# bcgsc/NanoSim

Measured on AMD Instinct MI355X. Metric: simulated reads/sec (genome mode, mean 8 kb), higher is better.
Workload: dtype u8

## Files before the change

nanosim_amd/csrc/nanosim_amd.hip:

```cpp
#include <hip/hip_runtime.h>
#include <hipcub/hipcub.hpp>
#include <stdio.h>
#include <stdlib.h>
#include <string.h>
#include <algorithm>
#include <chrono>
#include <atomic>
#include <condition_variable>
#include <functional>
#include <mutex>
#include <thread>
#include <string>
#include <vector>

#include "ns_device.h"
#include "ns_materialise.h"
#include "ns_chain.h"
#include "ns_hp.h"
#include "ns_ir.h"
#include "ns_io.h"
#include "ns_pack.h"
#include "ns_cs_hist.h"

#ifndef NS_WPB
// ... 3044 lines not shown
            continue;
        }
        pl.tot_cap = cap;
        break;
    }
    A.pieces = (ns_piece *)ctx->pieces.p;
    A.key_pos = (const uint32_t *)ctx->key_pos.p;
    pl.tot_pieces = n;
    info->ms_kernel[NS_K_EVENTS] = ms_chain;
    if (A.ir_need && (rc = ir_splice(ctx, A, n))) return rc;
    if (A.hp && (rc = hp_stage1(ctx, prm, A, n, pl.tot_pieces, stats, &pl.ms_hp))) return rc;
    return NS_OK;
}

static int genome_passes(ns_ctx *ctx, const ns_params *prm, ns_batch_info *info, GenArgs &A, Plan &pl) {
    const size_t n = (size_t)prm->n_reads;
    const Knobs &kn = ctx->knob;
    hipStream_t st = ctx->stream;
    unsigned long long *stats = pl.stats;
    uint32_t *list_a = (uint32_t *)ctx->order.p, *list_b = (uint32_t *)ctx->list_b.p, *list_c = (uint32_t *)ctx->list_c.p;
    const dim3 blk(256), grid_t((unsigned)((n + 1 + 255) / 256));
    const bool lds = ctx->lds_tables && prm->kind != NS_KIND_PERFECT;
    const bool chim_al = prm->kind == NS_KIND_ALIGNED && prm->chimeric;
    int rc;
    A.cap_rate = ctx->cap_rate;
    for (int hp_round = 0;; ++hp_round) {
        for (int retry = 0;; ++retry) {
            HIPCHK(hipMemsetAsync(ctx->stats.p, 0, NS_STATS_BYTES, st));
            HIPCHK(hipEventRecord(ctx->evt[1], st));
            k_nseg<<<grid_t, blk, 0, st>>>(A);
            HIPCHK(hipGetLastError());
            if ((rc = scan_u32(ctx, A.n_pieces, A.piece_off, n + 1))) return rc;
            if (chim_al) {
                uint32_t tp32 = 0;
                if ((rc = read_small(ctx, st, &tp32, A.piece_off + n, 4))) return rc;
                pl.tot_pieces = tp32;
            } else pl.tot_pieces = n;
            if ((rc = ensure(ctx, ctx->pieces, (size_t)pl.tot_pieces * sizeof(ns_piece) + 64))) return rc;
            A.pieces = (ns_piece *)ctx->pieces.p;
            A.list = nullptr; A.list_n = (uint32_t)n; A.attempt = 0;
            k_lengths<false><<<grid_t, blk, 0, st>>>(A);
            HIPCHK(hipGetLastError());
            if ((rc = scan_u64(ctx, A.ev_cap, A.ev_off, n + 1))) return rc;
            if ((rc = visiting_order(ctx, A.sort_key, A.sort_idx, n, list_a))) return rc;
            HIPCHK(hipEventRecord(ctx->evt[2], st));
            uint32_t n_multi = 0;
            if (prm->chimeric && prm->kind == NS_KIND_ALIGNED && ctx->ord_bins.p && !kn.exact_order) {
                if ((rc = read_small(ctx, st, &pl.tot_cap, A.ev_off + n, 8, &n_multi, (uint32_t *)ctx->ord_bins.p + 2 * NS_ORD_BINS, 4))) return rc;
            } else if ((rc = read_small(ctx, st, &pl.tot_cap, A.ev_off + n, 8))) return rc;
            if ((rc = ensure(ctx, ctx->events, (size_t)pl.tot_cap * sizeof(ns_event) + 64))) return rc;
            A.events = (ns_event *)ctx->events.p;
            uint32_t *cur = list_a, *nxt = list_b;
            uint32_t cur_n = (uint32_t)n;
            bool overflow = false;
            double ms_chain = 0;
            uint64_t used = pl.tot_cap;
            for (uint32_t a = 0;; ++a) {
                A.list = cur; A.list_n = cur_n; A.attempt = a; A.next_list = nxt; A.hole_at = 0; A.hole_len = 0; A.prio_thr = nullptr;
                A.l_off = nullptr; A.l_base = 0;
                if (a > 0) HIPCHK(hipMemsetAsync(A.next_n, 0, 4, st));
                const dim3 grid_p((cur_n + 255) / 256);
                A.p_need = nullptr; A.p_off = nullptr; A.p_base = 0;
                if (a > 0) {
                    if (chim_al) {
                        if ((rc = ensure_all(ctx, {{ctx->p_need, ((size_t)cur_n + 1) * 4}, {ctx->p_off, ((size_t)cur_n + 1) * 4}}))) return rc;
                        k_replan<<<dim3((cur_n + 1 + 255) / 256), blk, 0, st>>>(A, (uint32_t *)ctx->p_need.p);
                        HIPCHK(hipGetLastError());
                        if ((rc = scan_u32(ctx, (const uint32_t *)ctx->p_need.p, (uint32_t *)ctx->p_off.p, (size_t)cur_n + 1))) return rc;
                        uint32_t extra = 0;
                        if ((rc = read_small(ctx, st, &extra, (uint32_t *)ctx->p_off.p + cur_n, 4))) return rc;
                        if (extra) {
                            if ((rc = ensure_keep(ctx, ctx->pieces, (size_t)(pl.tot_pieces + extra) * sizeof(ns_piece) + 64,
                                                  (size_t)pl.tot_pieces * sizeof(ns_piece)))) return rc;
                            A.pieces = (ns_piece *)ctx->pieces.p;
                            A.p_need = (const uint32_t *)ctx->p_need.p; A.p_off = (const uint32_t *)ctx->p_off.p; A.p_base = (uint32_t)pl.tot_pieces;
                            pl.tot_pieces += extra;
                        }
                    }
                    if (cur_n <= 4096u) k_lengths<true><<<dim3((cur_n + 63) / 64), dim3(64), 0, st>>>(A);
                    else k_lengths<false><<<grid_p, blk, 0, st>>>(A);
                    HIPCHK(hipGetLastError());
                    HIPCHK(hipMemsetAsync(A.l_cap + cur_n, 0, 8, st));
                    if ((rc = scan_u64(ctx, A.l_cap, (uint64_t *)ctx->l_off.p, (size_t)cur_n + 1))) return rc;
                    uint64_t pass_cap = 0;
                    if ((rc = read_small(ctx, st, &pass_cap, (uint64_t *)ctx->l_off.p + cur_n, 8))) return rc;
                    if ((rc = ensure_keep(ctx, ctx->events, (size_t)(used + pass_cap) * sizeof(ns_event) + 64, (size_t)used * sizeof(ns_event)))) return rc;
                    A.events = (ns_event *)ctx->events.p;
                    A.l_off = (const uint64_t *)ctx->l_off.p; A.l_base = used;
                    used += pass_cap;
                }
                if (a == 0 && ctx->gate_wait) {
                    const auto t_end = std::chrono::steady_clock::now() + std::chrono::milliseconds(3);
                    while (!ctx->gate_wait->load(std::memory_order_acquire) && std::chrono::steady_clock::now() < t_end)
                        std::this_thread::yield();
                }
                HIPCHK(hipEventRecord(ctx->evt[3], st));
                uint32_t n_coop = 0;
                if (prm->kind == NS_KIND_UNALIGNED)
                    n_coop = (a == 0 && lds && cur_n >= kn.coop_min) ? std::max(cur_n >> kn.ucoop_shift, 1u) : cur_n;
                else if (a == 0 && ctx->coop_ok && prm->kind == NS_KIND_ALIGNED && cur_n >= kn.coop_min)
                    n_coop = (cur_n - std::min(cur_n, n_multi)) >> kn.coop_shift;
                const uint32_t coop_at = (a == 0 && prm->kind == NS_KIND_ALIGNED) ? std::min(cur_n, n_multi) : 0u;
                uint32_t m_coop = 0;
                if (coop_at && n_coop) {
                    const bool piece_threads = lds && !kn.no_piece_threads;
                    const uint32_t sh = piece_threads ? (kn.coop_shift > 1u ? kn.coop_shift - 1u : 0u) : (kn.coop_shift > 5u ? kn.coop_shift - 5u : 0u);
                    m_coop = std::min(coop_at, std::max(coop_at >> sh, 64u));
                }
                if (n_coop) {
                    GenArgs B = A; B.list_n = n_coop + m_coop; B.list = cur + (m_coop ? 0u : coop_at);
                    if (m_coop) { B.hole_at = m_coop; B.hole_len = coop_at - m_coop; }
                    B.coop_k1 = kn.ucoop_k1 ? 1u : 0u;
                    if ((rc = launch_chain_coop(ctx, B, st))) return rc;
                    if (coop_at) { A.list = cur + m_coop; A.hole_at = coop_at - m_coop; A.hole_len = n_coop; } else A.list = cur + n_coop;
                    A.list_n = cur_n - n_coop - m_coop;
                }
                uint32_t n_pt = 0;
                if (a == 0 && lds && n_coop && coop_at > m_coop && !kn.no_piece_threads) {
                    if (!ctx->stream3) {
                        HIPCHK(hipStreamCreateWithFlags(&ctx->stream3, hipStreamNonBlocking));
                        HIPCHK(hipEventCreateWithFlags(&ctx->ev_join3, hipEventDisableTiming));
                    }
                    n_pt = coop_at - m_coop;
                    const uint32_t cb = ctx->chain_block;
                    GenArgs P = A; P.list = cur + m_coop; P.list_n = n_pt; P.hole_at = 0; P.hole_len = 0; P.prio_thr = nullptr;
                    const size_t lds_p = ctx->lds_bytes + (P.ev_stage ? cb * 32u : 0u);
                    HIPCHK(hipStreamWaitEvent(ctx->stream3, ctx->ev_fork, 0));
                    P.piece_mode = 1;
                    k_chain<true, false, true><<<dim3((unsigned)(((uint64_t)n_pt * NS_PIECE_SLOTS + cb - 1) / cb)), dim3(cb), lds_p, ctx->stream3>>>(P);
                    P.piece_mode = 2;
                    k_chain<true, false, true><<<dim3((n_pt + cb - 1) / cb), dim3(cb), lds_p, ctx->stream3>>>(P);
                    HIPCHK(hipGetLastError());
                    HIPCHK(hipEventRecord(ctx->ev_join3, ctx->stream3));
                    A.list = cur + coop_at + n_coop; A.hole_at = 0; A.hole_len = 0; A.list_n = cur_n - coop_at - n_coop;
                }
                if (a == 0 && n_multi && !n_pt && prm->kind == NS_KIND_ALIGNED) A.prio_thr = (const uint32_t *)ctx->ord_bins.p + 2 * NS_ORD_BINS;
                if ((rc = launch_chain(ctx, A, st))) return rc;
                if (n_coop) HIPCHK(hipStreamWaitEvent(st, ctx->ev_join, 0));
                if (n_pt) HIPCHK(hipStreamWaitEvent(st, ctx->ev_join3, 0));
                HIPCHK(hipEventRecord(ctx->evt[4], st));
                if (ctx->gate_signal) ctx->gate_signal->store(1, std::memory_order_release);
                if ((rc = end_pass(ctx, A, retry, stats, ms_chain, info, overflow))) return rc;
                if (overflow) break;
                cur_n = (uint32_t)(stats[6] & 0xffffffffull);
                if (!cur_n) { pl.tot_cap = used; break; }
                if (a + 1 >= NS_MAX_ATTEMPT) return attempt_limit(ctx);
                cur = nxt; nxt = cur == list_b ? list_c : list_b;
            }
            info->ms_kernel[NS_K_EVENTS] = ms_chain;
#ifdef NS_CHAIN_CLOCK
            if (prm->kind == NS_KIND_ALIGNED) { unsigned long long c[16], z[16] = {0}; HIPCHK(hipMemcpyFromSymbol(c, HIP_SYMBOL(g_chain_clock), sizeof c)); HIPCHK(hipMemcpyToSymbol(HIP_SYMBOL(g_chain_clock), z, sizeof z));
              fprintf(stderr, "chain clock: lane 0 of the multi waves: aligned pieces %.3f ms, gaps %.3f ms, behind the lists %.3f ms (means) | ", c[6] ? c[8] * 1e-5 / c[6] : 0.0, c[6] ? c[9] * 1e-5 / c[6] : 0.0, c[6] ? c[10] * 1e-5 / c[6] : 0.0);
              fprintf(stderr, "chain clock: single waves %llu max %.3f ms mean %.3f ms (the group's last block: %llu) | multi waves %llu max %.3f ms mean %.3f ms (the group's last block: %llu) | ms_chain %.3f\n",
                  c[2], c[0] * 1e-5, c[2] ? c[1] * 1e-5 / c[2] : 0.0, c[3] >> 32, c[6], c[4] * 1e-5, c[6] ? c[5] * 1e-5 / c[6] : 0.0, c[7] >> 32, ms_chain); }
#endif
            if (!overflow) break;
        }
        if (A.ir_need && (rc = ir_splice(ctx, A, n))) return rc;
        if (!A.hp) break;
        if ((rc = hp_stage1(ctx, prm, A, n, pl.tot_pieces, stats, &pl.ms_hp))) return rc;
        if (!stats[5]) break;
        if (hp_round >= (int)NS_MAX_ATTEMPT) return fail(ctx, NS_EINVAL, "reads keep failing the final length check in -k mode");
        A.keep_state = 1;
    }
    return NS_OK;
}

static int check_params(ns_ctx *ctx, const ns_params *prm) {
    if (!ctx->has_model || !ctx->has_ref) return fail(ctx, NS_ESTATE, "ns_generate before ns_load_model/ns_set_reference");
    if (prm->kind > NS_KIND_PERFECT) return fail(ctx, NS_EINVAL, "bad kind");
    if (prm->emit_records > NS_EMIT_SIZES) return fail(ctx, NS_EINVAL, "bad emit_records");
    if (prm->kind != NS_KIND_PERFECT && !(ctx->m.flags & NS_MODEL_HAS_ERRORS)) return fail(ctx, NS_EINVAL, "model has no error tables");
    if (prm->kind == NS_KIND_UNALIGNED && !prm->use_lognormal && !(ctx->m.flags & NS_MODEL_HAS_UNALIGNED))
        return fail(ctx, NS_EINVAL, "model has no unaligned-length KDE");
    if (prm->fastq && !(ctx->m.flags & NS_MODEL_HAS_QUALS)) return fail(ctx, NS_EINVAL, "model has no quality tables");
    if (prm->chimeric && !(ctx->m.flags & NS_MODEL_HAS_CHIMERIC)) return fail(ctx, NS_EINVAL, "model has no chimeric tables");
    if (prm->kmer_bias && prm->kind == NS_KIND_ALIGNED && !(ctx->m.flags & NS_MODEL_HAS_HP))
        return fail(ctx, NS_EINVAL, "-k needs the homopolymer model (-hp)");
    const bool meta_al = prm->meta && prm->kind != NS_KIND_UNALIGNED;
    if (prm->meta) {
        if (!ctx->nspecies) return fail(ctx, NS_ESTATE, "metagenome batch before ns_set_species");
        if (prm->kind == NS_KIND_PERFECT && prm->chimeric) return fail(ctx, NS_EINVAL, "perfect reads cannot be chimeric");
        if (meta_al && !ctx->has_abun) return fail(ctx, NS_ESTATE, "metagenome batch before ns_set_abundance");
        if (meta_al && prm->chimeric && !ctx->has_inflated) return fail(ctx, NS_EINVAL, "chimeric metagenome batch needs abun_inflated");
    }
    if (prm->trx) {
        if (!ctx->has_trx) return fail(ctx, NS_ESTATE, "transcriptome batch before ns_set_transcriptome");
        if (prm->meta || prm->chimeric || prm->use_lognormal) return fail(ctx, NS_EINVAL, "transcriptome batches are neither metagenome nor chimeric nor log-normal");
        if (prm->kind != NS_KIND_UNALIGNED && !(ctx->m.flags & NS_MODEL_HAS_KDE2D)) return fail(ctx, NS_EINVAL, "model has no 2-D KDE (_aligned_region_2d)");
    }
    if (prm->model_ir) {
        if (!prm->trx) return fail(ctx, NS_EINVAL, "model_ir is a transcriptome option");
        if (!ctx->has_ir) return fail(ctx, NS_ESTATE, "model_ir batch before ns_set_intron_retention");
    }
    if (prm->n_reads > 0x7ffffff0ull) return fail(ctx, NS_EINVAL, "batch too large (split into several calls)");
    if (prm->first_read + prm->n_reads >= (1ull << 40)) return fail(ctx, NS_EINVAL, "read index exceeds 2^40");
    return NS_OK;
}

static int batch_args(ns_ctx *ctx, const ns_params *prm, size_t n, GenArgs &A) {
    int rc;
    if ((rc = ensure_all(ctx, {{ctx->n_pieces, (n + 1) * 4}, {ctx->piece_off, (n + 1) * 4}, {ctx->ev_cap, (n + 1) * 8}, {ctx->ev_off, (n + 1) * 8},
                               {ctx->l_cap, (n + 1) * 8}, {ctx->l_off, (n + 1) * 8}, {ctx->rec_len, (n + 1) * 8}, {ctx->rec_off, (n + 1) * 8},
                               {ctx->err_len, (n + 1) * 8}, {ctx->err_off, (n + 1) * 8}, {ctx->name_len, (n + 1) * 2}, {ctx->reads, n * sizeof(ns_read)},
                               {ctx->stats, NS_STATS_BYTES}, {ctx->sort_key, (n + 1) * 4}, {ctx->sort_idx, (n + 1) * 4}, {ctx->sort_key_out, (n + 1) * 4},
                               {ctx->order, (n + 1) * 4}, {ctx->list_b, (n + 1) * 4}, {ctx->list_c, (n + 1) * 4}, {ctx->rstate, (n + 1) * 4},
                               {ctx->att_base, (n + 1) * 4}, {ctx->scr_len, (n + 1) * 8}, {ctx->scr_off, (n + 1) * 8}})))
        return rc;
    memset(&A, 0, sizeof A);
    A.prm = *prm; A.m = ctx->m; A.ref = ctx->ref;
    A.key_first = A.name_first = prm->first_read;
    A.cap_gap_mul = 2;
    A.ev_stage = (ctx->lds_tables && ctx->lds_bytes + ctx->chain_block * 32u <= 64u * 1024u) ? (uint32_t)ctx->lds_bytes : 0u;
    A.n_pieces = (uint32_t *)ctx->n_pieces.p; A.piece_off = (uint32_t *)ctx->piece_off.p;
    A.ev_cap = (uint64_t *)ctx->ev_cap.p; A.ev_off = (uint64_t *)ctx->ev_off.p; A.l_cap = (uint64_t *)ctx->l_cap.p;
    A.rec_len = (uint64_t *)ctx->rec_len.p; A.rec_off = (uint64_t *)ctx->rec_off.p;
    A.err_len = (uint64_t *)ctx->err_len.p; A.err_off = (uint64_t *)ctx->err_off.p;
    A.name_len = (uint16_t *)ctx->name_len.p; A.reads = (ns_read *)ctx->reads.p;
    A.stats = (unsigned long long *)ctx->stats.p;
    A.sort_key = (uint32_t *)ctx->sort_key.p; A.sort_idx = (uint32_t *)ctx->sort_idx.p;
    A.rstate = (uint32_t *)ctx->rstate.p; A.att_base = (uint32_t *)ctx->att_base.p;
    A.scr_len = (uint64_t *)ctx->scr_len.p; A.scr_off = (uint64_t *)ctx->scr_off.p;
    A.hp = (prm->kmer_bias && prm->kind == NS_KIND_ALIGNED) ? 1u : 0u;
    A.errlen_later = prm->emit_errlog ? 1u : 0u;
    A.dbg = ctx->knob.dbg;
    if (prm->trx) {
        if ((rc = ensure(ctx, ctx->polya, (n + 1) * 2))) return rc;
        A.tx = ctx->tx; A.polya = (uint16_t *)ctx->polya.p;
        HIPCHK(hipMemsetAsync(ctx->polya.p, 0, (n + 1) * 2, ctx->stream));
    }
    ctx->spliced_bytes = 0;
    if (prm->model_ir && prm->kind == NS_KIND_ALIGNED) {
        if ((rc = ensure_all(ctx, {{ctx->ir_need, (n + 1) * 8}, {ctx->ir_off, (n + 1) * 8}}))) return rc;
        A.ir = ctx->ir; A.ir_need = (uint64_t *)ctx->ir_need.p;
    }
    A.meta = prm->meta ? 1u : 0u; A.nspecies = ctx->nspecies; A.species_chrom_off = (const uint32_t *)ctx->species_chrom_off.p;
    A.next_n = (uint32_t *)((unsigned long long *)ctx->stats.p + 6);
    return NS_OK;
}

static int write_images(ns_ctx *ctx, const ns_params *prm, ns_batch_info *info, GenArgs &A, const Plan &pl, bool meta_al,
                        const uint32_t *order, int *slot) {
    const size_t n = (size_t)prm->n_reads;
    hipStream_t st = ctx->stream;
    int rc;
    if (A.errlen_later && !A.hp && !meta_al) {
        k_errlen<<<dim3((unsigned)((n + NS_WPB - 1) / NS_WPB)), dim3(64 * NS_WPB), 0, st>>>(A);
        HIPCHK(hipGetLastError());
    }
    if ((rc = scan_u64(ctx, A.rec_len, A.rec_off, n + 1))) return rc;
    if (prm->emit_errlog && (rc = scan_u64(ctx, A.err_len, A.err_off, n + 1))) return rc;
    if ((rc = prm->emit_errlog ? read_small(ctx, st, &info->record_bytes, A.rec_off + n, 8, &info->errlog_bytes, A.err_off + n, 8)
                               : read_small(ctx, st, &info->record_bytes, A.rec_off + n, 8))) return rc;
    *slot = ctx->slot;
    const bool write_rec = prm->emit_records == 1u;
    if (write_rec && ctx->io) {
        if (ctx->io->slot_busy(*slot)) *slot ^= 1;
        ctx->io->wait_slot(*slot);
    }
    if (write_rec && (rc = ensure_all(ctx, {{ctx->rec_slot[*slot], (size_t)info->record_bytes + 64}, {ctx->err_slot[*slot], (size_t)info->errlog_bytes + 64}})))
        return rc;
    if (prm->emit_records == 0) info->errlog_bytes = 0;
    A.records = (uint8_t *)ctx->rec_slot[*slot].p; A.errlog = (uint8_t *)ctx->err_slot[*slot].p;
    A.cls = nullptr;
    if (write_rec && prm->fastq && prm->kind != NS_KIND_UNALIGNED) {
        const size_t per_read = prm->chimeric ? 2u * (2u * NS_MAX_SEG - 1u) : 2u;
        if ((rc = ensure(ctx, ctx->cls, (((size_t)info->record_bytes >> 4) + per_read * (n + 1) + 64) * 4))) return rc;
        A.cls = (uint32_t *)ctx->cls.p;
    }
    const uint64_t max_unaligned = prm->kind == NS_KIND_UNALIGNED ? pl.stats[1] : 0;
    HIPCHK(hipEventRecord(ctx->evt[5], st));
    if (write_rec) {
        HIPCHK(hipEventRecord(ctx->ev_fork, st));
        HIPCHK(hipStreamWaitEvent(ctx->stream2, ctx->ev_fork, 0));
    }
    k_names<<<dim3((unsigned)((n + 1 + 255) / 256)), dim3(256), 0, write_rec ? ctx->stream2 : st>>>(A);
    HIPCHK(hipGetLastError());
    if (write_rec) HIPCHK(hipEventRecord(ctx->ev_join, ctx->stream2));
    HIPCHK(hipEventRecord(ctx->evt[6], st));
    if (A.hp) {
        if (write_rec && (rc = launch_materialise(ctx, A, n, prm->fastq != 0, order, MAT_HP_FINAL))) return rc;
        k_hp_report<<<dim3((unsigned)((pl.tot_pieces + 255) / 256)), dim3(256), 0, st>>>(A, pl.tot_pieces);
        HIPCHK(hipGetLastError());
    } else if (write_rec) {
        if ((rc = launch_materialise(ctx, A, n, prm->fastq != 0, order, MAT_REF, max_unaligned))) return rc;
    }
    if (write_rec) HIPCHK(hipStreamWaitEvent(st, ctx->ev_join, 0));
    HIPCHK(hipEventRecord(ctx->evt[7], st));
    if (prm->emit_errlog && write_rec) {
        const uint64_t rows = pl.stats[3] ? pl.stats[3] : 1;
        if ((info->errlog_bytes / rows + 5) * 64 <= NS_ERR_BUF_SMALL) k_errlog<NS_ERR_BUF_SMALL><<<dim3((unsigned)n), dim3(64), 0, st>>>(A);
        else k_errlog<NS_ERR_BUF_LARGE><<<dim3((unsigned)n), dim3(64), 0, st>>>(A);
        HIPCHK(hipGetLastError());
    }
    HIPCHK(hipEventRecord(ctx->evt[8], st));
    return NS_OK;
}

static int finish_call(ns_ctx *ctx, const ns_params *prm, ns_batch_info *info, const Plan &pl, int slot) {
    float ms = 0;
    HIPCHK(hipStreamSynchronize(ctx->stream));
    HIPCHK(hipEventElapsedTime(&ms, ctx->evt[0], ctx->evt[8])); info->ms_total = ms;
    HIPCHK(hipEventElapsedTime(&ms, ctx->evt[1], ctx->evt[2])); info->ms_kernel[NS_K_LENGTHS] = ms;
    HIPCHK(hipEventElapsedTime(&ms, ctx->evt[5], ctx->evt[6])); info->ms_kernel[NS_K_SCAN] = ms;
    HIPCHK(hipEventElapsedTime(&ms, ctx->evt[6], ctx->evt[7])); info->ms_kernel[NS_K_MATERIALISE] = ms;
    HIPCHK(hipEventElapsedTime(&ms, ctx->evt[7], ctx->evt[8])); info->ms_kernel[NS_K_ERRLOG] = ms;
    if (ctx->rec_timed) { HIPCHK(hipEventElapsedTime(&ms, ctx->evt[12], ctx->evt[13])); info->ms_kernel[NS_K_RECORD_KERNEL] = ms; }
// ... 350 lines not shown
```

nanosim_amd/csrc/ns_chain.h:

```cpp
#pragma once
#include "ns_device.h"

struct Tabs {
    const uint64_t *w;
    NS_DEV const double *d(uint32_t off) const { return reinterpret_cast<const double *>(w + off); }
    NS_DEV const uint64_t *q(uint32_t off) const { return w + off; }
    NS_DEV const uint16_t *h(uint32_t off) const { return reinterpret_cast<const uint16_t *>(w + off); }
    NS_DEV const uint32_t *u(uint32_t off) const { return reinterpret_cast<const uint32_t *>(w + off); }
    NS_DEV const int32_t *i(uint32_t off) const { return reinterpret_cast<const int32_t *>(w + off); }
};

template <class V>
NS_DEV int32_t ecdf_lookup_g(const double *__restrict__ hi, const V *__restrict__ vhi, uint32_t n,
                                                 double vlo0, const uint16_t *__restrict__ guide, uint32_t u) {
    double p = u32_to_p(u);
    uint32_t s = guide[u >> 24];
    if (s < n) {
        const double h0 = hi[s], h1 = hi[min(s + 1, n - 1)];
        if (p > h0) {
            ++s;
            if (s < n && p > h1) { ++s; while (s < n && p > hi[s]) ++s; }
        }
    }
    if (s >= n) { s = n - 1; p = hi[s]; }
// ... 372 lines not shown
                    ty0 = NS_DEL; ln0 = step > L ? step - L : 1u; n_ev = 1;
                    if (L > step - 1) { ty1 = NS_INS; ln1 = L - (step - 1); n_ev = 2; }
                }
            }
        }
        bool bad = ln0 > NS_EV_LEN_MAX || ln1 > NS_EV_LEN_MAX || ln2 > NS_EV_LEN_MAX;
        ln0 = min(ln0, NS_EV_LEN_MAX); ln1 = min(ln1, NS_EV_LEN_MAX); ln2 = min(ln2, NS_EV_LEN_MAX);
        auto dsh = [](uint32_t ty, uint32_t ln) { return ty == NS_INS ? ln : ty == NS_DEL ? 0u - ln : 0u; };
        const uint32_t d0 = n_ev > 0 ? dsh(ty0, ln0) : 0u, d1 = n_ev > 1 ? dsh(ty1, ln1) : 0u;
        const uint32_t dn_incl = wave_incl_scan(del | n_ev << 24);
        const uint32_t del_incl = dn_incl & 0xffffffu, n_incl = dn_incl >> 24;
        const uint32_t slot = s.n + n_incl - n_ev;
        const uint32_t sh = (uint32_t)s.shift + (pend0 + ins_incl - L) - (del_incl - del);
        if ((n_ev > 0 && !ev_shift_fits((int32_t)sh)) || (n_ev > 1 && !ev_shift_fits((int32_t)(sh + d0))) || (n_ev > 2 && !ev_shift_fits((int32_t)(sh + d0 + d1)))) bad = true;
        if (__ballot(bad)) s.range = true;
        if (n_ev > 0) { if (slot < s.cap) { ns_event e; e.pos = ps0; e.info = ns_ev_pack(ln0, ty0, (int32_t)sh); s.ev[slot] = e; } }
        if (n_ev > 1) { if (slot + 1 < s.cap) { ns_event e; e.pos = ps1; e.info = ns_ev_pack(ln1, ty1, (int32_t)(sh + d0)); s.ev[slot + 1] = e; } }
        if (n_ev > 2) { if (slot + 2 < s.cap) { ns_event e; e.pos = ps2; e.info = ns_ev_pack(ln2, ty2, (int32_t)(sh + d0 + d1)); s.ev[slot + 2] = e; } }
        const uint32_t n_blk = (uint32_t)__builtin_amdgcn_readlane((int)n_incl, 63);
        if (s.n + n_blk > s.cap) s.overflow = true;
        s.n += n_blk;
        const uint32_t ins_tot = (uint32_t)__builtin_amdgcn_readlane((int)ins_incl, 63);
        const uint32_t del_tot = (uint32_t)__builtin_amdgcn_readlane((int)del_incl, 63);
        l_new += (int32_t)ins_tot - (int32_t)del_tot;
        const uint32_t pend1 = NB ? ins_tot - (uint32_t)__shfl((int)ins_incl, 63 - __clzll((long long)NB)) : pend0 + ins_tot;
        s.shift = (int32_t)((uint32_t)s.shift + (pend0 + ins_tot - pend1) - del_tot);
        pend0 = pend1;
        pos0 += (uint32_t)__builtin_amdgcn_readlane((int)adv_incl, (int)(n_exec - 1u));
        if (n_exec < 64 || pos0 >= (uint32_t)m_ref) break;
    }
    if ((int32_t)pos0 > middle_ref) { l_new += (int32_t)pos0 - middle_ref; middle_ref = (int32_t)pos0; }
    return EList32{l_new, middle_ref};
}

template <int K>
__device__ inline EList32 coopk_unaligned_error_list(const Tabs &T, const ChainTab &c, int32_t m_ref, const ns_key &key, uint32_t seg,
                                                     uint32_t attempt, EvSink32 &s, uint32_t lane) {
    int32_t l_new = m_ref, middle_ref = m_ref;
    if (m_ref <= 0) return EList32{l_new, middle_ref};
    uint32_t pos0 = 0, pend0 = 0;
    auto draw = [&](uint32_t it, int &type, uint32_t &step) {
        const u32x4 w = ns_draw(key, ST_UEVENT, seg, attempt, it, 0);
        const uint64_t ut = w.x;
        type = (ut < ns_thr_lt(0.4)) ? 3 : (ut < ns_thr_lt(0.7)) ? NS_MIS : (ut < ns_thr_lt(0.85)) ? NS_INS : NS_DEL;
        step = 1;
        if (type != 3) step = (uint32_t)run_length_t(T, c, type, w.y, w.z);
    };
    int type_n[K]; uint32_t step_n[K];
    #pragma unroll
    for (int k = 0; k < K; ++k) draw(lane * K + k, type_n[k], step_n[k]);
    bool bad = false;
    for (uint32_t it0 = 0;; it0 += 64u * K) {
        int type[K]; uint32_t step[K];
        #pragma unroll
        for (int k = 0; k < K; ++k) { type[k] = type_n[k]; step[k] = step_n[k]; }
        #pragma unroll
        for (int k = 0; k < K; ++k) draw(it0 + 64u * K + lane * K + k, type_n[k], step_n[k]);
        uint32_t a_loc[K], a_lane = 0;
        #pragma unroll
        for (int k = 0; k < K; ++k) { a_loc[k] = a_lane; a_lane += type[k] == NS_INS ? 0u : step[k]; }
        const uint32_t a_incl = wave_incl_scan(a_lane);
        const uint32_t pos_l = pos0 + a_incl - a_lane;
        bool exec[K], nonins[K], first[K];
        uint32_t L_loc[K], i_loc[K], d_loc[K], run = 0, i_lane = 0, d_lane = 0, a_exec = 0, n_exec_l = 0;
        bool seen = false;
        #pragma unroll
        for (int k = 0; k < K; ++k) {
            exec[k] = pos_l + a_loc[k] < (uint32_t)m_ref;
            if (!exec[k]) { step[k] = 0; type[k] = 3; }
            nonins[k] = exec[k] && type[k] != NS_INS;
            const uint32_t ins = (exec[k] && type[k] == NS_INS) ? step[k] : 0u, del = (exec[k] && type[k] == NS_DEL) ? step[k] : 0u;
            i_loc[k] = i_lane; d_loc[k] = d_lane;
            i_lane += ins; d_lane += del;
            run += ins;
            L_loc[k] = nonins[k] ? run : 0u;
            first[k] = nonins[k] && !seen;
            if (nonins[k]) { run = 0; seen = true; }
            a_exec += (exec[k] && type[k] != NS_INS) ? step[k] : 0u;
            n_exec_l += exec[k] ? 1u : 0u;
        }
        const uint32_t i_incl = wave_incl_scan(i_lane);
        const uint64_t HAS = __ballot(seen);
        const uint64_t below = HAS & ((1ull << lane) - 1ull);
        const int jb = below ? 63 - __clzll((long long)below) : (int)lane;
        const uint32_t tail_b = (uint32_t)__shfl((int)run, jb), incl_b = (uint32_t)__shfl((int)i_incl, jb);
        const uint32_t pend_l = below ? tail_b + (i_incl - i_lane) - incl_b : pend0 + (i_incl - i_lane);
        uint32_t ty[K][3], ln[K][3], ps[K][3], n_ev[K], n_loc[K], L[K], n_lane = 0;
        #pragma unroll
        for (int k = 0; k < K; ++k) {
            const uint32_t pos = pos_l + a_loc[k], st = step[k];
            L[k] = nonins[k] ? L_loc[k] + (first[k] ? pend_l : 0u) : 0u;
            const uint32_t Lk = L[k];
            ty[k][0] = ty[k][1] = ty[k][2] = 0; ln[k][0] = ln[k][1] = ln[k][2] = 0; ps[k][0] = pos; ps[k][1] = ps[k][2] = pos + 1;
            uint32_t ne = 0;
            if (nonins[k]) {
                if (type[k] == 3) { if (Lk) { ty[k][0] = NS_INS; ln[k][0] = Lk; ps[k][0] = pos + 1; ne = 1; } }
                else if (type[k] == NS_MIS) {
                    if (!Lk) { ty[k][0] = NS_MIS; ln[k][0] = st; ne = 1; }
                    else {
                        ty[k][0] = NS_MIS; ln[k][0] = 1; ty[k][1] = NS_INS; ln[k][1] = Lk; ne = 2;
                        if (st - 1 > Lk) { ty[k][2] = NS_MIS; ln[k][2] = st - 1 - Lk; ne = 3; }
                    }
                } else {
                    if (!Lk) { ty[k][0] = NS_DEL; ln[k][0] = st; ne = 1; }
                    else {
                        ty[k][0] = NS_DEL; ln[k][0] = st > Lk ? st - Lk : 1u; ne = 1;
                        if (Lk > st - 1) { ty[k][1] = NS_INS; ln[k][1] = Lk - (st - 1); ne = 2; }
                    }
                }
            }
            bad |= ln[k][0] > NS_EV_LEN_MAX || ln[k][1] > NS_EV_LEN_MAX || ln[k][2] > NS_EV_LEN_MAX;
            ln[k][0] = min(ln[k][0], NS_EV_LEN_MAX); ln[k][1] = min(ln[k][1], NS_EV_LEN_MAX); ln[k][2] = min(ln[k][2], NS_EV_LEN_MAX);
            n_ev[k] = ne; n_loc[k] = n_lane; n_lane += ne;
        }
        const uint32_t d_incl = wave_incl_scan(d_lane);
        const uint32_t ne_incl = wave_incl_scan(n_lane | n_exec_l << 16);
        const uint32_t d_front = d_incl - d_lane, n_front = (ne_incl & 0xffffu) - n_lane;
        auto dsh = [](uint32_t t, uint32_t l) { return t == NS_INS ? l : t == NS_DEL ? 0u - l : 0u; };
        #pragma unroll
        for (int k = 0; k < K; ++k) {
            if (!n_ev[k]) continue;
            const uint32_t sh = (uint32_t)s.shift + (pend0 + (i_incl - i_lane) + i_loc[k] - L[k]) - (d_front + d_loc[k]);
            const uint32_t d0 = dsh(ty[k][0], ln[k][0]), d1 = n_ev[k] > 1 ? dsh(ty[k][1], ln[k][1]) : 0u;
            if (!ev_shift_fits((int32_t)sh) || (n_ev[k] > 1 && !ev_shift_fits((int32_t)(sh + d0))) || (n_ev[k] > 2 && !ev_shift_fits((int32_t)(sh + d0 + d1)))) bad = true;
            const uint32_t slot = s.n + n_front + n_loc[k];
            if (slot < s.cap) { ns_event e; e.pos = ps[k][0]; e.info = ns_ev_pack(ln[k][0], ty[k][0], (int32_t)sh); s.ev[slot] = e; }
            if (n_ev[k] > 1 && slot + 1 < s.cap) { ns_event e; e.pos = ps[k][1]; e.info = ns_ev_pack(ln[k][1], ty[k][1], (int32_t)(sh + d0)); s.ev[slot + 1] = e; }
            if (n_ev[k] > 2 && slot + 2 < s.cap) { ns_event e; e.pos = ps[k][2]; e.info = ns_ev_pack(ln[k][2], ty[k][2], (int32_t)(sh + d0 + d1)); s.ev[slot + 2] = e; }
        }
        const uint32_t ne_tot = (uint32_t)__builtin_amdgcn_readlane((int)ne_incl, 63);
        const uint32_t n_blk = ne_tot & 0xffffu, n_ran = ne_tot >> 16;
        const uint32_t del_tot = (uint32_t)__builtin_amdgcn_readlane((int)d_incl, 63), ins_tot = (uint32_t)__builtin_amdgcn_readlane((int)i_incl, 63);
        uint32_t adv_tot = (uint32_t)__builtin_amdgcn_readlane((int)a_incl, 63);
        if (n_ran < 64u * K) adv_tot = (uint32_t)__builtin_amdgcn_readlane((int)wave_incl_scan(a_exec), 63);
        if (s.n + n_blk > s.cap) s.overflow = true;
        s.n += n_blk;
        l_new += (int32_t)ins_tot - (int32_t)del_tot;
        uint32_t pend1 = pend0 + ins_tot;
        if (HAS) {
            const int jl = 63 - __clzll((long long)HAS);
            pend1 = (uint32_t)__shfl((int)run, jl) + ins_tot - (uint32_t)__shfl((int)i_incl, jl);
        }
        s.shift = (int32_t)((uint32_t)s.shift + (pend0 + ins_tot - pend1) - del_tot);
        pend0 = pend1;
        pos0 += adv_tot;
        if (n_ran < 64u * K || pos0 >= (uint32_t)m_ref) break;
    }
    if (__ballot(bad)) s.range = true;
    if ((int32_t)pos0 > middle_ref) { l_new += (int32_t)pos0 - middle_ref; middle_ref = (int32_t)pos0; }
    return EList32{l_new, middle_ref};
}

#define COOP_MAX_BINS 16u
struct CoopLds {
    uint32_t err_tab[64];
    uint16_t step_tab[64][4];
    uint32_t match_tab[64][COOP_MAX_BINS];
    ns_event ev_buf[64];
};

__device__ inline EList32 coop_error_list(const Tabs &TM, const Tabs &T, const ChainTab &c, int32_t m_ref, const ns_key &key, uint32_t seg,
                                          uint32_t attempt, EvSink32 &s, CoopLds &S, uint32_t lane) {
    int32_t l_new = m_ref, pos = 0, middle_ref = m_ref;
    int state = NS_ST_START;
    u32x4 w = ns_draw(key, ST_EVENT, seg, attempt, 0, 0);
    int32_t prev_match = ecdf_lookup_g(T.d(c.fm_hi), T.d(c.fm_vhi), c.fm_n, c.fm_vlo0, T.h(c.fm_guide), w.x);
    if (prev_match < 2) prev_match = 2;
    pos += prev_match;
    uint32_t it0 = 1;
    int32_t last_ins_pos = -1;
    const uint64_t *trans = TM.q(c.trans);
    const int32_t *bins = T.i(c.mm_bin);
    const uint32_t *seg_off = T.u(c.mm_seg_off);
    const uint8_t *bin_lut = reinterpret_cast<const uint8_t *>(T.w + c.mm_bin_lut);
    auto bin_of = [&](int32_t v) -> uint32_t {
        if ((uint32_t)v < 256u) return bin_lut[v];
        uint32_t b = 0;
        for (; b < c.mm_nbins; ++b)
            if (bins[2 * b] <= v && v < bins[2 * b + 1]) break;
        return b >= c.mm_nbins ? c.mm_nbins - 1 : b;
    };
    uint32_t pbin = bin_of(prev_match);
    while (pos < middle_ref) {
        {
            const u32x4 wi = ns_draw(key, ST_EVENT, seg, attempt, it0 + lane, 0);
            uint32_t eb = 0;
#pragma unroll
            for (int st = 0; st < 7; ++st) eb |= (uint32_t)trans_pick_u(trans + 3 * st, wi.x) << (2 * st);
            S.err_tab[lane] = eb;
#pragma unroll
            for (int t = 0; t < 3; ++t) S.step_tab[lane][t] = (uint16_t)run_length_t(TM, c, t, wi.y, wi.z);
            if (c.int_image) {
                const uint16_t *g16 = T.h(c.mm_g16);
                const uint64_t *gvf = T.q(c.mm_gv_full);
                const uint32_t cell = wi.w >> 16, nb = c.mm_nbins;
                const uint64_t uu = wi.w;
                for (uint32_t b0 = 0; b0 < nb; b0 += 4) {
                    uint32_t o[4], nc[4], s0[4];
                    uint64_t ga[4], gb[4];
#pragma unroll
                    for (uint32_t k = 0; k < 4; ++k) {
                        const uint32_t b = min(b0 + k, nb - 1u);
                        o[k] = seg_off[b]; nc[k] = seg_off[b + 1] - o[k];
                        s0[k] = g16[(size_t)b * 65536u + cell];
                    }
#pragma unroll
                    for (uint32_t k = 0; k < 4; ++k) {
                        const uint32_t sc = min(s0[k], nc[k] ? nc[k] - 1u : 0u);
                        ga[k] = gvf[o[k] + sc]; gb[k] = gvf[o[k] + sc + 1u];
                    }
#pragma unroll
                    for (uint32_t k = 0; k < 4; ++k) {
                        const uint32_t b = min(b0 + k, nb - 1u);
                        const uint32_t k0 = (s0[k] < nc[k] ? 1u : 0u) & (uu >= NS_G_THR(ga[k]) ? 1u : 0u);
                        const uint32_t k1 = k0 & (s0[k] + 1u < nc[k] ? 1u : 0u) & (uu >= NS_G_THR(gb[k]) ? 1u : 0u);
                        const uint64_t g = k0 ? gb[k] : ga[k];
                        int32_t v = (int32_t)(uint32_t)(g >> 35) - 1;
                        if (!((s0[k] + k0 < nc[k]) && !k1 && (g & NS_GV_UNIT)))
                            v = ecdf_lookup_gv(gvf + o[k], nc[k], T.h(c.mm_guide) + 256u * b, wi.w, T.q(c.sub2_full), T.d(c.mm_hi) + o[k], T.d(c.mm_vhi) + o[k], T.d(c.mm_vlo0)[b]);
                        if (b0 + k < nb) S.match_tab[lane][b0 + k] = (uint32_t)(uint16_t)v | bin_of(v) << 16 | bin_of(v == 0 ? 1 : v) << 24;
                    }
                }
            } else
            for (uint32_t b = 0; b < c.mm_nbins; ++b) {
                const uint32_t o = seg_off[b];
                const int32_t v = ecdf_lookup_g(T.d(c.mm_hi) + o, T.d(c.mm_vhi) + o, seg_off[b + 1] - o, T.d(c.mm_vlo0)[b], T.h(c.mm_guide) + 256 * b, wi.w);
                S.match_tab[lane][b] = (uint32_t)(uint16_t)v | bin_of(v) << 16 | bin_of(v == 0 ? 1 : v) << 24;
            }
        }
        __builtin_amdgcn_fence(__ATOMIC_ACQ_REL, "wavefront");
        __builtin_amdgcn_wave_barrier();
        uint32_t nl = 0;
        uint32_t i = 0;
        for (; i < 64 && pos < middle_ref; ++i) {
            const int error = (int)((S.err_tab[i] >> (2 * state)) & 3u);
            int32_t step = S.step_tab[i][error];
            if (error == NS_INS) l_new += step; else if (error == NS_DEL) l_new -= step;
            int32_t epos = pos;
            if (error != NS_INS) {
                pos += step;
                if (pos >= middle_ref) { l_new += pos - middle_ref; middle_ref = pos; }
            } else {
                if (last_ins_pos == pos && (nl > 0 || s.n > 0)) {
                    if (nl > 0) --nl; else --s.n;
                    s.shift -= (int32_t)s.last_ins_len;
                }
                last_ins_pos = pos;
            }
            {
                const uint32_t l = step > (int32_t)NS_EV_LEN_MAX ? NS_EV_LEN_MAX : (uint32_t)step;
                if (step > (int32_t)NS_EV_LEN_MAX || !ev_shift_fits(s.shift)) s.range = true;
                ns_event e; e.pos = (uint32_t)epos; e.info = ns_ev_pack(l, (uint32_t)error, s.shift);
                if (lane == 0) S.ev_buf[nl] = e;
                ++nl;
                if (error == NS_INS) { s.shift += (int32_t)l; s.last_ins_len = l; } else if (error == NS_DEL) s.shift -= (int32_t)l;
            }
            state = NS_ST_MIS + error;
            const uint32_t me = S.match_tab[i][pbin];
            step = (int32_t)(me & 0xffffu);
            pbin = (me >> 16) & 0xffu;
            if (prev_match == 0 && step == 0) { step = 1; pbin = me >> 24; }
            prev_match = step;
            if (pos + prev_match > middle_ref) { l_new += pos + prev_match - middle_ref; middle_ref = pos + prev_match; }
            pos += prev_match;
            if (prev_match == 0) state += 3;
            else last_ins_pos = -1;
        }
        __builtin_amdgcn_fence(__ATOMIC_ACQ_REL, "wavefront");
        __builtin_amdgcn_wave_barrier();
        if (lane < nl) {
            if (s.n + lane < s.cap) s.ev[s.n + lane] = S.ev_buf[lane];
        }
        if (s.n + nl > s.cap) s.overflow = true;
        s.n += nl;
        it0 += i;
        __builtin_amdgcn_fence(__ATOMIC_ACQ_REL, "wavefront");
        __builtin_amdgcn_wave_barrier();
    }
    return EList32{l_new, middle_ref};
}
```

Before: 126.2 million.

## Replace serial per-lane event walk with wave-parallel scan over state maps

The cooperative error-list walk previously had each lane speculate draws and then walked 64 steps serially on every lane. It now composes per-step bin-transition maps and 7-state error-state maps with a log-step parallel prefix in LDS and registers, then uses wave scans for positions, shifts, kept events and length deltas so that all 64 steps resolve in parallel. Events are written directly from their lanes instead of through a lane-0 staging buffer. This adds LDS traffic and compose work (log2(64) rounds over up to 5 words of byte maps) and more complex insertion-collapse logic, which carries a correctness risk.

Measured after the change: 128.2 million (median of 6 runs). Within noise of the previous version (+1.6%).

```diff
diff --git a/nanosim_amd/csrc/nanosim_amd.hip b/nanosim_amd/csrc/nanosim_amd.hip
--- a/nanosim_amd/csrc/nanosim_amd.hip
+++ b/nanosim_amd/csrc/nanosim_amd.hip
@@ -3220,7 +3220,9 @@
             if (prm->kind == NS_KIND_ALIGNED) { unsigned long long c[16], z[16] = {0}; HIPCHK(hipMemcpyFromSymbol(c, HIP_SYMBOL(g_chain_clock), sizeof c)); HIPCHK(hipMemcpyToSymbol(HIP_SYMBOL(g_chain_clock), z, sizeof z));
               fprintf(stderr, "chain clock: lane 0 of the multi waves: aligned pieces %.3f ms, gaps %.3f ms, behind the lists %.3f ms (means) | ", c[6] ? c[8] * 1e-5 / c[6] : 0.0, c[6] ? c[9] * 1e-5 / c[6] : 0.0, c[6] ? c[10] * 1e-5 / c[6] : 0.0);
               fprintf(stderr, "chain clock: single waves %llu max %.3f ms mean %.3f ms (the group's last block: %llu) | multi waves %llu max %.3f ms mean %.3f ms (the group's last block: %llu) | ms_chain %.3f\n",
-                  c[2], c[0] * 1e-5, c[2] ? c[1] * 1e-5 / c[2] : 0.0, c[3] >> 32, c[6], c[4] * 1e-5, c[6] ? c[5] * 1e-5 / c[6] : 0.0, c[7] >> 32, ms_chain); }
+                  c[2], c[0] * 1e-5, c[2] ? c[1] * 1e-5 / c[2] : 0.0, c[3] >> 32, c[6], c[4] * 1e-5, c[6] ? c[5] * 1e-5 / c[6] : 0.0, c[7] >> 32, ms_chain);
+              unsigned long long w[4], wz[4] = {0}; HIPCHK(hipMemcpyFromSymbol(w, HIP_SYMBOL(g_coop_clock), sizeof w)); HIPCHK(hipMemcpyToSymbol(HIP_SYMBOL(g_coop_clock), wz, sizeof wz));
+              if (w[2]) fprintf(stderr, "chain clock: wave-per-read list, the wavefront of its first read: %llu blocks, speculation %.2f us + walk %.2f us per block\n", w[2], w[0] * 1e-2 / w[2], w[1] * 1e-2 / w[2]); }
 #endif
             if (!overflow) break;
         }
diff --git a/nanosim_amd/csrc/ns_chain.h b/nanosim_amd/csrc/ns_chain.h
--- a/nanosim_amd/csrc/ns_chain.h
+++ b/nanosim_amd/csrc/ns_chain.h
@@ -548,23 +548,42 @@
 }
 
 #define COOP_MAX_BINS 16u
+#define COOP_MAP_WORDS 5u
 struct CoopLds {
     uint32_t err_tab[64];
     uint16_t step_tab[64][4];
     uint32_t match_tab[64][COOP_MAX_BINS];
-    ns_event ev_buf[64];
+    uint32_t amap[64][COOP_MAP_WORDS];
 };
 
-__device__ inline EList32 coop_error_list(const Tabs &TM, const Tabs &T, const ChainTab &c, int32_t m_ref, const ns_key &key, uint32_t seg,
-                                          uint32_t attempt, EvSink32 &s, CoopLds &S, uint32_t lane) {
-    int32_t l_new = m_ref, pos = 0, middle_ref = m_ref;
-    int state = NS_ST_START;
-    u32x4 w = ns_draw(key, ST_EVENT, seg, attempt, 0, 0);
-    int32_t prev_match = ecdf_lookup_g(T.d(c.fm_hi), T.d(c.fm_vhi), c.fm_n, c.fm_vlo0, T.h(c.fm_guide), w.x);
-    if (prev_match < 2) prev_match = 2;
-    pos += prev_match;
-    uint32_t it0 = 1;
-    int32_t last_ins_pos = -1;
+#ifdef NS_HOST_TEST
+#define NS_WAVE_FN inline
+#define NS_EACH_LANE(l, lane) for (uint32_t l = 0; l < 64u; ++l)
+template <class T> struct WaveVar { T v[64]; T &operator[](uint32_t l) { return v[l]; } const T &operator[](uint32_t l) const { return v[l]; } };
+inline void wv_sync() {}
+inline void wv_scan_add(WaveVar<uint32_t> &x) { for (uint32_t l = 1; l < 64u; ++l) x.v[l] += x.v[l - 1]; }
+inline uint64_t wv_ballot(const WaveVar<uint32_t> &x) { uint64_t b = 0; for (uint32_t l = 0; l < 64u; ++l) b |= (uint64_t)(x.v[l] != 0u) << l; return b; }
+inline uint32_t wv_read(const WaveVar<uint32_t> &x, uint32_t src) { return x.v[src & 63u]; }
+inline void wv_shift_up(WaveVar<uint32_t> &out, const WaveVar<uint32_t> &x, uint32_t d, uint32_t fill) {
+    for (uint32_t l = 64u; l-- > 0u;) out.v[l] = l >= d ? x.v[l - d] : fill;
+}
+#else
+#define NS_WAVE_FN __device__ inline
+#define NS_EACH_LANE(l, lane) for (uint32_t l = (lane), ns_once_ = 1u; ns_once_; ns_once_ = 0u)
+template <class T> struct WaveVar { T v; __device__ T &operator[](uint32_t) { return v; } __device__ const T &operator[](uint32_t) const { return v; } };
+__device__ inline void wv_sync() { __builtin_amdgcn_fence(__ATOMIC_ACQ_REL, "wavefront"); __builtin_amdgcn_wave_barrier(); }
+__device__ inline void wv_scan_add(WaveVar<uint32_t> &x) { x.v = wave_incl_scan(x.v); }
+__device__ inline uint64_t wv_ballot(const WaveVar<uint32_t> &x) { return __ballot(x.v != 0u); }
+__device__ inline uint32_t wv_read(const WaveVar<uint32_t> &x, uint32_t src) { return (uint32_t)__builtin_amdgcn_readlane((int)x.v, (int)(src & 63u)); }
+__device__ inline void wv_shift_up(WaveVar<uint32_t> &out, const WaveVar<uint32_t> &x, uint32_t d, uint32_t fill) {
+    const uint32_t l = __lane_id();
+    const uint32_t y = (uint32_t)__shfl((int)x.v, (int)((l - d) & 63u));
+    out.v = l >= d ? y : fill;
+}
+#endif
+
+NS_DEV void coop_speculate(const Tabs &TM, const Tabs &T, const ChainTab &c, const ns_key &key, uint32_t seg, uint32_t attempt, uint32_t it,
+                           CoopLds &S, uint32_t lane) {
     const uint64_t *trans = TM.q(c.trans);
     const int32_t *bins = T.i(c.mm_bin);
     const uint32_t *seg_off = T.u(c.mm_seg_off);
@@ -576,102 +595,210 @@
             if (bins[2 * b] <= v && v < bins[2 * b + 1]) break;
         return b >= c.mm_nbins ? c.mm_nbins - 1 : b;
     };
-    uint32_t pbin = bin_of(prev_match);
-    while (pos < middle_ref) {
-        {
-            const u32x4 wi = ns_draw(key, ST_EVENT, seg, attempt, it0 + lane, 0);
-            uint32_t eb = 0;
+    const u32x4 wi = ns_draw(key, ST_EVENT, seg, attempt, it, 0);
+    uint32_t eb = 0;
 #pragma unroll
-            for (int st = 0; st < 7; ++st) eb |= (uint32_t)trans_pick_u(trans + 3 * st, wi.x) << (2 * st);
-            S.err_tab[lane] = eb;
+    for (int st = 0; st < 7; ++st) eb |= (uint32_t)trans_pick_u(trans + 3 * st, wi.x) << (2 * st);
+    S.err_tab[lane] = eb;
 #pragma unroll
-            for (int t = 0; t < 3; ++t) S.step_tab[lane][t] = (uint16_t)run_length_t(TM, c, t, wi.y, wi.z);
-            if (c.int_image) {
-                const uint16_t *g16 = T.h(c.mm_g16);
-                const uint64_t *gvf = T.q(c.mm_gv_full);
-                const uint32_t cell = wi.w >> 16, nb = c.mm_nbins;
-                const uint64_t uu = wi.w;
-                for (uint32_t b0 = 0; b0 < nb; b0 += 4) {
-                    uint32_t o[4], nc[4], s0[4];
-                    uint64_t ga[4], gb[4];
+    for (int t = 0; t < 3; ++t) S.step_tab[lane][t] = (uint16_t)run_length_t(TM, c, t, wi.y, wi.z);
+    if (c.int_image) {
+        const uint16_t *g16 = T.h(c.mm_g16);
+        const uint64_t *gvf = T.q(c.mm_gv_full);
+        const uint32_t cell = wi.w >> 16, nb = c.mm_nbins;
+        const uint64_t uu = wi.w;
+        for (uint32_t b0 = 0; b0 < nb; b0 += 4) {
+            uint32_t o[4], nc[4], s0[4];
+            uint64_t ga[4], gb[4];
 #pragma unroll
-                    for (uint32_t k = 0; k < 4; ++k) {
-                        const uint32_t b = min(b0 + k, nb - 1u);
-                        o[k] = seg_off[b]; nc[k] = seg_off[b + 1] - o[k];
-                        s0[k] = g16[(size_t)b * 65536u + cell];
+            for (uint32_t k = 0; k < 4; ++k) {
+                const uint32_t b = min(b0 + k, nb - 1u);
+                o[k] = seg_off[b]; nc[k] = seg_off[b + 1] - o[k];
+                s0[k] = g16[(size_t)b * 65536u + cell];
+            }
+#pragma unroll
+            for (uint32_t k = 0; k < 4; ++k) {
+                const uint32_t sc = min(s0[k], nc[k] ? nc[k] - 1u : 0u);
+                ga[k] = gvf[o[k] + sc]; gb[k] = gvf[o[k] + sc + 1u];
+            }
+#pragma unroll
+            for (uint32_t k = 0; k < 4; ++k) {
+                const uint32_t b = min(b0 + k, nb - 1u);
+                const uint32_t k0 = (s0[k] < nc[k] ? 1u : 0u) & (uu >= NS_G_THR(ga[k]) ? 1u : 0u);
+                const uint32_t k1 = k0 & (s0[k] + 1u < nc[k] ? 1u : 0u) & (uu >= NS_G_THR(gb[k]) ? 1u : 0u);
+                const uint64_t g = k0 ? gb[k] : ga[k];
+                int32_t v = (int32_t)(uint32_t)(g >> 35) - 1;
+                if (!((s0[k] + k0 < nc[k]) && !k1 && (g & NS_GV_UNIT)))
+                    v = ecdf_lookup_gv(gvf + o[k], nc[k], T.h(c.mm_guide) + 256u * b, wi.w, T.q(c.sub2_full), T.d(c.mm_hi) + o[k], T.d(c.mm_vhi) + o[k], T.d(c.mm_vlo0)[b]);
+                if (b0 + k < nb) S.match_tab[lane][b0 + k] = (uint32_t)(uint16_t)v | bin_of(v) << 16 | bin_of(v == 0 ? 1 : v) << 24;
+            }
+        }
+    } else
+    for (uint32_t b = 0; b < c.mm_nbins; ++b) {
+        const uint32_t o = seg_off[b];
+        const int32_t v = ecdf_lookup_g(T.d(c.mm_hi) + o, T.d(c.mm_vhi) + o, seg_off[b + 1] - o, T.d(c.mm_vlo0)[b], T.h(c.mm_guide) + 256 * b, wi.w);
+        S.match_tab[lane][b] = (uint32_t)(uint16_t)v | bin_of(v) << 16 | bin_of(v == 0 ? 1 : v) << 24;
+    }
+}
+
+#if defined(NS_CHAIN_CLOCK) && !defined(NS_HOST_TEST)
+__device__ unsigned long long g_coop_clock[4];
+#define COOP_CLOCK(x) x
+#else
+#define COOP_CLOCK(x)
+#endif
+struct CoopWalk {
+    uint32_t state;
+    uint32_t a;
+    int32_t pos, last_ins_pos;
+};
+NS_DEV uint32_t coop_map7_compose(uint32_t first, uint32_t then) {
+    uint32_t r = 0;
+#pragma unroll
+    for (uint32_t st = 0; st < 7u; ++st) r |= ((then >> (3u * ((first >> (3u * st)) & 7u))) & 7u) << (3u * st);
+    return r;
+}
+#define COOP_MAP7_ID 0x1ac688u
+NS_WAVE_FN uint32_t coop_walk_block(CoopLds &S, uint32_t nbins, uint32_t bin0, int32_t m_ref, CoopWalk &W, EvSink32 &s, int32_t &l_new, uint32_t lane) {
+    (void)lane;
+    const uint32_t nw = (nbins + 4u) >> 2;
+    NS_EACH_LANE(l, lane) {
+        uint8_t *row = reinterpret_cast<uint8_t *>(S.amap[l]);
+        for (uint32_t a = 0; a < 4u * nw; ++a) {
+            const uint32_t me = S.match_tab[l][a < nbins ? a : bin0];
+            uint32_t o = (me & 0xffffu) ? (me >> 16) & 0xffu : nbins;
+            if (a == nbins && !(me & 0xffffu)) o = me >> 24;
+            row[a] = (uint8_t)(a <= nbins ? o : 0u);
+        }
+    }
+    wv_sync();
+    for (uint32_t d = 1; d < 64u; d <<= 1) {
+        WaveVar<uint32_t> r0, r1, r2, r3, r4;
+        NS_EACH_LANE(l, lane) {
+            const uint32_t *own = S.amap[l];
+            uint32_t r[COOP_MAP_WORDS] = {own[0], own[1], own[2], own[3], own[4]};
+            if (l >= d) {
+                const uint32_t *low = S.amap[l - d];
+                const uint8_t *ob = reinterpret_cast<const uint8_t *>(own);
+#pragma unroll
+                for (uint32_t w = 0; w < COOP_MAP_WORDS; ++w)
+                    if (w < nw) {
+                        const uint32_t e = low[w];
+                        r[w] = (uint32_t)ob[e & 0xffu] | (uint32_t)ob[(e >> 8) & 0xffu] << 8 | (uint32_t)ob[(e >> 16) & 0xffu] << 16 | (uint32_t)ob[e >> 24] << 24;
                     }
+            }
+            r0[l] = r[0]; r1[l] = r[1]; r2[l] = r[2]; r3[l] = r[3]; r4[l] = r[4];
+        }
+        wv_sync();
+        NS_EACH_LANE(l, lane) { uint32_t *own = S.amap[l]; own[0] = r0[l]; own[1] = r1[l]; own[2] = r2[l]; own[3] = r3[l]; own[4] = r4[l]; }
+        wv_sync();
+    }
+    WaveVar<uint32_t> m, zero_m, map7, eb;
+    NS_EACH_LANE(l, lane) {
+        const uint32_t a_in = l ? reinterpret_cast<const uint8_t *>(S.amap[l - 1])[W.a] : W.a;
+        const uint32_t me = S.match_tab[l][a_in < nbins ? a_in : bin0];
+        uint32_t mv = me & 0xffffu;
+        if (a_in == nbins && mv == 0u) mv = 1u;
+        m[l] = mv; zero_m[l] = mv == 0u ? 1u : 0u;
+        const uint32_t e = S.err_tab[l];
+        uint32_t q = 0;
 #pragma unroll
-                    for (uint32_t k = 0; k < 4; ++k) {
-                        const uint32_t sc = min(s0[k], nc[k] ? nc[k] - 1u : 0u);
-                        ga[k] = gvf[o[k] + sc]; gb[k] = gvf[o[k] + sc + 1u];
-                    }
-#pragma unroll
-                    for (uint32_t k = 0; k < 4; ++k) {
-                        const uint32_t b = min(b0 + k, nb - 1u);
-                        const uint32_t k0 = (s0[k] < nc[k] ? 1u : 0u) & (uu >= NS_G_THR(ga[k]) ? 1u : 0u);
-                        const uint32_t k1 = k0 & (s0[k] + 1u < nc[k] ? 1u : 0u) & (uu >= NS_G_THR(gb[k]) ? 1u : 0u);
-                        const uint64_t g = k0 ? gb[k] : ga[k];
-                        int32_t v = (int32_t)(uint32_t)(g >> 35) - 1;
-                        if (!((s0[k] + k0 < nc[k]) && !k1 && (g & NS_GV_UNIT)))
-                            v = ecdf_lookup_gv(gvf + o[k], nc[k], T.h(c.mm_guide) + 256u * b, wi.w, T.q(c.sub2_full), T.d(c.mm_hi) + o[k], T.d(c.mm_vhi) + o[k], T.d(c.mm_vlo0)[b]);
-                        if (b0 + k < nb) S.match_tab[lane][b0 + k] = (uint32_t)(uint16_t)v | bin_of(v) << 16 | bin_of(v == 0 ? 1 : v) << 24;
-                    }
-                }
-            } else
-            for (uint32_t b = 0; b < c.mm_nbins; ++b) {
-                const uint32_t o = seg_off[b];
-                const int32_t v = ecdf_lookup_g(T.d(c.mm_hi) + o, T.d(c.mm_vhi) + o, seg_off[b + 1] - o, T.d(c.mm_vlo0)[b], T.h(c.mm_guide) + 256 * b, wi.w);
-                S.match_tab[lane][b] = (uint32_t)(uint16_t)v | bin_of(v) << 16 | bin_of(v == 0 ? 1 : v) << 24;
-            }
-        }
-        __builtin_amdgcn_fence(__ATOMIC_ACQ_REL, "wavefront");
-        __builtin_amdgcn_wave_barrier();
-        uint32_t nl = 0;
-        uint32_t i = 0;
-        for (; i < 64 && pos < middle_ref; ++i) {
-            const int error = (int)((S.err_tab[i] >> (2 * state)) & 3u);
-            int32_t step = S.step_tab[i][error];
-            if (error == NS_INS) l_new += step; else if (error == NS_DEL) l_new -= step;
-            int32_t epos = pos;
-            if (error != NS_INS) {
-                pos += step;
-                if (pos >= middle_ref) { l_new += pos - middle_ref; middle_ref = pos; }
-            } else {
-                if (last_ins_pos == pos && (nl > 0 || s.n > 0)) {
-                    if (nl > 0) --nl; else --s.n;
-                    s.shift -= (int32_t)s.last_ins_len;
-                }
-                last_ins_pos = pos;
-            }
-            {
-                const uint32_t l = step > (int32_t)NS_EV_LEN_MAX ? NS_EV_LEN_MAX : (uint32_t)step;
-                if (step > (int32_t)NS_EV_LEN_MAX || !ev_shift_fits(s.shift)) s.range = true;
-                ns_event e; e.pos = (uint32_t)epos; e.info = ns_ev_pack(l, (uint32_t)error, s.shift);
-                if (lane == 0) S.ev_buf[nl] = e;
-                ++nl;
-                if (error == NS_INS) { s.shift += (int32_t)l; s.last_ins_len = l; } else if (error == NS_DEL) s.shift -= (int32_t)l;
-            }
-            state = NS_ST_MIS + error;
-            const uint32_t me = S.match_tab[i][pbin];
-            step = (int32_t)(me & 0xffffu);
-            pbin = (me >> 16) & 0xffu;
-            if (prev_match == 0 && step == 0) { step = 1; pbin = me >> 24; }
-            prev_match = step;
-            if (pos + prev_match > middle_ref) { l_new += pos + prev_match - middle_ref; middle_ref = pos + prev_match; }
-            pos += prev_match;
-            if (prev_match == 0) state += 3;
-            else last_ins_pos = -1;
-        }
-        __builtin_amdgcn_fence(__ATOMIC_ACQ_REL, "wavefront");
-        __builtin_amdgcn_wave_barrier();
-        if (lane < nl) {
-            if (s.n + lane < s.cap) s.ev[s.n + lane] = S.ev_buf[lane];
-        }
-        if (s.n + nl > s.cap) s.overflow = true;
-        s.n += nl;
-        it0 += i;
-        __builtin_amdgcn_fence(__ATOMIC_ACQ_REL, "wavefront");
-        __builtin_amdgcn_wave_barrier();
+        for (uint32_t st = 0; st < 7u; ++st) q |= ((uint32_t)NS_ST_MIS + ((e >> (2u * st)) & 3u) + (mv == 0u ? 3u : 0u)) << (3u * st);
+        eb[l] = e; map7[l] = q;
+    }
+    for (uint32_t d = 1; d < 64u; d <<= 1) {
+        WaveVar<uint32_t> low;
+        wv_shift_up(low, map7, d, COOP_MAP7_ID);
+        NS_EACH_LANE(l, lane) map7[l] = coop_map7_compose(low[l], map7[l]);
+    }
+    WaveVar<uint32_t> map7_low;
+    wv_shift_up(map7_low, map7, 1, COOP_MAP7_ID);
+    WaveVar<uint32_t> error, step, adv, pos_in, exec;
+    NS_EACH_LANE(l, lane) {
+        const uint32_t st = (map7_low[l] >> (3u * W.state)) & 7u;
+        error[l] = (eb[l] >> (2u * st)) & 3u;
+        step[l] = S.step_tab[l][error[l]];
+        adv[l] = (error[l] == (uint32_t)NS_INS ? 0u : step[l]) + m[l];
+    }
+    WaveVar<uint32_t> adv_incl = adv;
+    wv_scan_add(adv_incl);
+    NS_EACH_LANE(l, lane) {
+        pos_in[l] = (uint32_t)W.pos + adv_incl[l] - adv[l];
+        exec[l] = (int32_t)pos_in[l] < m_ref ? 1u : 0u;
+    }
+    const uint32_t n_exec = (uint32_t)__builtin_popcountll(wv_ballot(exec));
+    WaveVar<uint32_t> ins_x, open_x;
+    NS_EACH_LANE(l, lane) {
+        ins_x[l] = exec[l] & (error[l] == (uint32_t)NS_INS ? 1u : 0u);
+        open_x[l] = exec[l] & (ins_x[l] | (zero_m[l] ^ 1u));
+    }
+    const uint64_t INS = wv_ballot(ins_x), ZM = wv_ballot(zero_m), OPEN = wv_ballot(open_x);
+    const bool coll_in = (INS & 1ull) && W.last_ins_pos == W.pos && s.n > 0u;
+    if (coll_in) { --s.n; s.shift -= (int32_t)s.last_ins_len; }
+    WaveVar<uint32_t> len, kept, dsh, dl;
+    NS_EACH_LANE(l, lane) {
+        const bool replaced = l < 63u && ins_x[l] && zero_m[l] && ((INS >> (l + 1u)) & 1ull);
+        kept[l] = exec[l] && !replaced ? 1u : 0u;
+        len[l] = step[l] > NS_EV_LEN_MAX ? NS_EV_LEN_MAX : step[l];
+        const uint32_t sgn = error[l] == (uint32_t)NS_INS ? len[l] : error[l] == (uint32_t)NS_DEL ? 0u - len[l] : 0u;
+        dsh[l] = kept[l] ? sgn : 0u;
+        dl[l] = !exec[l] ? 0u : error[l] == (uint32_t)NS_INS ? step[l] : error[l] == (uint32_t)NS_DEL ? 0u - step[l] : 0u;
+    }
+    WaveVar<uint32_t> kept_incl = kept, dsh_incl = dsh;
+    wv_scan_add(kept_incl); wv_scan_add(dsh_incl); wv_scan_add(dl);
+    WaveVar<uint32_t> bad;
+    NS_EACH_LANE(l, lane) {
+        const int32_t sh = s.shift + (int32_t)(dsh_incl[l] - dsh[l]);
+        bad[l] = exec[l] && (step[l] > NS_EV_LEN_MAX || !ev_shift_fits(sh)) ? 1u : 0u;
+        const uint32_t slot = s.n + kept_incl[l] - kept[l];
+        if (kept[l] && slot < s.cap) { ns_event e; e.pos = pos_in[l]; e.info = ns_ev_pack(len[l], error[l], sh); s.ev[slot] = e; }
+    }
+    if (wv_ballot(bad)) s.range = true;
+    const uint32_t last = n_exec - 1u;
+    s.n += wv_read(kept_incl, 63);
+    if (s.n > s.cap) s.overflow = true;
+    s.shift += (int32_t)wv_read(dsh_incl, 63);
+    l_new += (int32_t)wv_read(dl, 63);
+    if (INS) s.last_ins_len = wv_read(len, 63u - (uint32_t)__builtin_clzll(INS));
+    if (OPEN) {
+        const uint32_t h = 63u - (uint32_t)__builtin_clzll(OPEN);
+        W.last_ins_pos = ((ZM >> h) & 1ull) ? (int32_t)wv_read(pos_in, h) : -1;
+    }
+    W.pos += (int32_t)wv_read(adv_incl, last);
+    W.state = (wv_read(map7, 63) >> (3u * W.state)) & 7u;
+    W.a = reinterpret_cast<const uint8_t *>(S.amap[63])[W.a];
+    return n_exec;
+}
+
+NS_WAVE_FN EList32 coop_error_list(const Tabs &TM, const Tabs &T, const ChainTab &c, int32_t m_ref, const ns_key &key, uint32_t seg,
+                                   uint32_t attempt, EvSink32 &s, CoopLds &S, uint32_t lane) {
+    int32_t l_new = m_ref, middle_ref = m_ref;
+    u32x4 w = ns_draw(key, ST_EVENT, seg, attempt, 0, 0);
+    int32_t prev_match = ecdf_lookup_g(T.d(c.fm_hi), T.d(c.fm_vhi), c.fm_n, c.fm_vlo0, T.h(c.fm_guide), w.x);
+    if (prev_match < 2) prev_match = 2;
+    uint32_t it0 = 1;
+    const int32_t *bins = T.i(c.mm_bin);
+    const uint8_t *bin_lut = reinterpret_cast<const uint8_t *>(T.w + c.mm_bin_lut);
+    auto bin_of = [&](int32_t v) -> uint32_t {
+        if ((uint32_t)v < 256u) return bin_lut[v];
+        uint32_t b = 0;
+        for (; b < c.mm_nbins; ++b)
+            if (bins[2 * b] <= v && v < bins[2 * b + 1]) break;
+        return b >= c.mm_nbins ? c.mm_nbins - 1 : b;
+    };
+    CoopWalk W{(uint32_t)NS_ST_START, bin_of(prev_match), prev_match, -1};
+    const uint32_t bin0 = bin_of(0);
+    while (W.pos < middle_ref) {
+        COOP_CLOCK(const unsigned long long clk0 = wall_clock64();)
+        NS_EACH_LANE(l, lane) coop_speculate(TM, T, c, key, seg, attempt, it0 + l, S, l);
+        wv_sync();
+        COOP_CLOCK(const unsigned long long clk1 = wall_clock64();)
+        const uint32_t n = coop_walk_block(S, c.mm_nbins, bin0, m_ref, W, s, l_new, lane);
+        COOP_CLOCK(if (blockIdx.x == 0 && lane == 0) { atomicAdd(&g_coop_clock[0], clk1 - clk0); atomicAdd(&g_coop_clock[1], wall_clock64() - clk1); atomicAdd(&g_coop_clock[2], 1ull); })
+        it0 += n;
+        if (W.pos > middle_ref) { l_new += W.pos - middle_ref; middle_ref = W.pos; }
+        if (n < 64u) break;
+        wv_sync();
     }
     return EList32{l_new, middle_ref};
 }
```
